# google-deepmind/bsuite

Hardware: AMD Instinct MI355X
Metric: env-steps/sec (higher is better)
Workload: dtype int32; 1 GPU; deep_sea/10 deep_sea {'size': 30, 'mapping_seed': 42} random actions, dense TimeStep; mode=e, lanes_per_gpu=1048576, global_lanes=1048576, episode_phases=staggered

## Files before the change

### bsuite_amd/csrc/deep_sea.hip

```cpp
#include "bsx_pair_host.h"
#include "bsx_tab_eval.h"
#include "deep_sea_fam.h"
#include "pair_mixed.h"

template <int K>
__global__ void __launch_bounds__(BSX_BLOCK) deep_sea_step1_kernel(const deep_sea_fam::args a, const uint32_t cells,
                                                                   const uint32_t cells_magic, const bsx_div64 dv) {
  __shared__ deep_sea_fam::shared s_map[BSX_BLOCK / BSX_WAVE];
  const int wl = (int)(threadIdx.x & 63u);
  deep_sea_fam::shared& map = s_map[threadIdx.x >> 6];
  const int64_t n_lanes = a.ctl.n_lanes;
  const uint64_t step = bsx_step_of(a.ctl);
  const int32_t tag_new = (int32_t)(((uint32_t)(step + 1) & 1u) << DS_TAG_SHIFT);
  const bool forced = a.ctl.force_reset != 0;
  const deep_sea_hot fn{a.size};
  const uint64_t total = (uint64_t)n_lanes * cells;
  const uint64_t F0 = (uint64_t)blockIdx.x * (uint64_t)(K * 4 * BSX_BLOCK);
  const uint64_t lane_b = __umul64hi(F0, dv.m) >> dv.s;
  const uint32_t r_b = (uint32_t)(F0 - lane_b * cells);
  bsx_f4* __restrict__ o4 = reinterpret_cast<bsx_f4*>(a.out.observation + F0);
  const int32_t* __restrict__ st_b = a.state + lane_b;
  const int32_t* __restrict__ act_b = a.action + (forced ? 0 : lane_b);

  uint32_t dl[K];
  int r0[K];
  bool live[K];
#pragma unroll
  for (int u = 0; u < K; ++u) {
    const uint32_t c = (threadIdx.x >> 6) * (K * 64) + u * 64 + (threadIdx.x & 63);
    const uint32_t f = r_b + (c << 2);
    dl[u] = __umulhi(f, cells_magic);
    r0[u] = (int)(f - dl[u] * cells);
    live[u] = F0 + ((uint64_t)c << 2) + 3 < total;
  }
  const uint32_t dA = dl[0];
  uint32_t dB = dA;
  bool wrA = false, wrB = false;
#pragma unroll
  for (int u = 0; u < K; ++u) {
    if (live[u]) dB = dl[u];
  }
#pragma unroll
  for (int u = 0; u < K; ++u) {
    wrA |= live[u] && r0[u] == 0 && dl[u] == dA;
    wrB |= live[u] && r0[u] == 0 && dl[u] == dB && dB != dA;
  }
  const bool any = live[0];
  const int32_t wA = any ? st_b[dA] : 0, wB = any ? st_b[dB] : 0;
  const int aA = (any && !forced) ? act_b[dA] : 0, aB = (any && !forced) ? act_b[dB] : 0;

  const int map_words = (a.size * a.size + 31) >> 5;
  static_assert(DS_MAP_WORDS <= 2 * BSX_WAVE, "the per-wave copy of the action mapping is two passes at most");
  if (wl < map_words) map.map[wl] = a.mapping_bits[wl];
  if (wl + BSX_WAVE < map_words) map.map[wl + BSX_WAVE] = a.mapping_bits[wl + BSX_WAVE];
  bsx_wave_sync();


  auto resolve = [&](uint32_t d, int32_t w, int act, bool writer, int& type) -> int32_t {
    type = -1;
    if (!writer && (w & DS_TAG_BIT) == tag_new) return w;
    const int64_t L = (int64_t)lane_b + d;
    int32_t nst; double reward;
    const int ty = deep_sea_fam::advance<true, 1>(a, map, L, a.ctl.lane_offset + (uint64_t)L, step, w, act, nst, reward, writer);
    if (writer) {
      type = ty;
      a.state[L] = nst;
      bsx_emit_at<0, 0, false>(a.ctl, a.out, L, L, a.ctl.lane_offset + (uint64_t)L, step, ty, reward);
    }
    return nst;
  };
  int tA = -1, tB = -1;
  int32_t nA = 0, nB = 0;
  if (any) {
    nA = resolve(dA, wA, aA, wrA, tA);
    nB = dB != dA ? resolve(dB, wB, aB, wrB, tB) : nA;
  }
  int hA, hB, unused;
  fn(nA, hA, unused);
  fn(nB, hB, unused);
#pragma unroll
  for (int u = 0; u < K; ++u) {
    if (!live[u]) continue;
    int hot = dl[u] == dA ? hA : hB;
    const int p0 = hot < 0 ? -1 : hot - r0[u];
    bsx_f4 v;
    v.x = p0 == 0 ? 1.0f : 0.0f;
    v.y = p0 == 1 ? 1.0f : 0.0f;
    v.z = p0 == 2 ? 1.0f : 0.0f;
    v.w = p0 == 3 ? 1.0f : 0.0f;
    o4[(threadIdx.x >> 6) * (K * 64) + u * 64 + (threadIdx.x & 63)] = v;
  }
  const unsigned int n_last = (unsigned int)__popcll(__ballot(tA == BSX_LAST)) + (unsigned int)__popcll(__ballot(tB == BSX_LAST));
  const unsigned int n_first = (unsigned int)__popcll(__ballot(tA == BSX_FIRST)) + (unsigned int)__popcll(__ballot(tB == BSX_FIRST));
  if (a.ctl.counters != nullptr && wl == 0 && (n_last | n_first) != 0u) {
    unsigned long long* shard = (unsigned long long*)a.ctl.counters +
                                (size_t)((blockIdx.x * (BSX_BLOCK / BSX_WAVE) + (threadIdx.x >> 6)) & (BSX_COUNTER_SHARDS - 1)) * BSX_COUNTER_STRIDE;
    if (n_last) atomicAdd(&shard[0], (unsigned long long)n_last);
    if (n_first) atomicAdd(&shard[1], (unsigned long long)n_first);
  }
}

static int deep_sea_check_cfg(const bsx_deep_sea_t* cfg) {
  return (cfg->size < 1 || cfg->size > BSX_DEEP_SEA_MAX_SIZE) ? BSX_ERANGE : 0;
}

static void deep_sea_fill(const bsx_deep_sea_t* cfg, const bsx_call_t* call, const int32_t* action, int32_t* state,
                          bsx_timestep_t out, double* info, deep_sea_fam::args* a) {
  a->ctl = bsx_make_ctl(call);
  a->action = action; a->state = state; a->out = out; a->info = info;
  a->move_cost = cfg->move_cost; a->inv_size = cfg->inv_size;
  a->size = cfg->size; a->deterministic = cfg->deterministic;
  for (int w = 0; w < DS_MAP_WORDS; ++w) a->mapping_bits[w] = cfg->mapping_bits[w];
}

static int deep_sea_make(const bsx_deep_sea_t* cfg, const bsx_call_t* call, const int32_t* action,
                         int32_t* state, bsx_timestep_t out, double* info, deep_sea_fam::args* a) {
  if (cfg == nullptr) return BSX_ENULL;
  int rc = bsx_check_call(call, action, out, true, true);
  if (rc != 0) return rc;
  if ((rc = deep_sea_check_cfg(cfg)) != 0) return rc;
  if (call->stream.mt_state != nullptr && !cfg->deterministic && call->stream.mt_gauss == nullptr)
    return BSX_ENULL;
  if (call->n_lanes > 0 && (state == nullptr || info == nullptr)) return BSX_ENULL;
  deep_sea_fill(cfg, call, action, state, out, info, a);
  return 0;
}

extern "C" int bsx_deep_sea_step(const bsx_deep_sea_t* cfg, const bsx_call_t* call,
                                 const int32_t* action, int32_t* state, bsx_timestep_t out,
                                 double* info) {
  deep_sea_fam::args a;
  int rc = deep_sea_make(cfg, call, action, state, out, info, &a);
  if (rc != 0) return rc;
  if (call->n_lanes == 0) return 0;
  const uint32_t cells = (uint32_t)(cfg->size * cfg->size);
  static const int step1_env = bsx_env_int("BSX_DEEP_SEA_STEP1", 1);
  if (step1_env != 0 && (int64_t)call->n_lanes * cells * 4 <= ((int64_t)1 << 30) && (call->flags & BSX_CALL_STATE_TAGGED) && call->n_steps <= 1 && call->action_ring <= 1 && cfg->deterministic && bsx_ctl_lean(a.ctl) &&
      call->obs_paint == nullptr && bsx_call_obs(call) == 0 && !bsx_call_index(call) && (cells & 3u) == 0 && cells >= 3u * 256u) {
    constexpr int K = 4;
    const uint64_t total = (uint64_t)call->n_lanes * cells;
    const uint64_t blocks = (total + (uint64_t)K * 4 * BSX_BLOCK - 1) / ((uint64_t)K * 4 * BSX_BLOCK);
    if (blocks > 0x7FFFFFFFull) return BSX_EINVAL;
    deep_sea_step1_kernel<K><<<dim3((unsigned)blocks), dim3(BSX_BLOCK), 0, (hipStream_t)call->hip_stream>>>(
        a, cells, bsx_div_magic(cells), bsx_make_div64(cells));
    return bsx_launch_status();
  }
  return bsx_pair_call<deep_sea_fam, deep_sea_hot, 4>(a, call, action, state, out, cells, deep_sea_hot{cfg->size});
}

extern "C" int bsx_deep_sea_policy_rollout(const bsx_deep_sea_t* cfg, const bsx_call_t* call, const bsx_policy_t* policy,
                                           int32_t* state, bsx_timestep_t out, double* info) {
  if (cfg == nullptr || call == nullptr || policy == nullptr) return BSX_ENULL;
  int rc = deep_sea_check_cfg(cfg);
  if (rc == 0) rc = bsx_check_policy_call(call, policy, bsx_policy_states_deep_sea(cfg->size), state, out, info);
  if (rc != 0 || call->n_lanes == 0) return rc;
  deep_sea_fam::args a;
  rc = deep_sea_make(cfg, call, policy->actions_out, state, out, info, &a);
  if (rc != 0) return rc;
  a.action = nullptr;
  return bsx_policy_rollout_call<deep_sea_fam, deep_sea_hot>(a, call, policy, 2u, out, deep_sea_hot{cfg->size});
}

extern "C" int bsx_deep_sea_policy_evaluate(const bsx_deep_sea_t* cfg, const bsx_call_t* call, const bsx_policy_t* policy,
                                             int32_t* state, bsx_policy_eval_t out, double* info) {
  if (cfg == nullptr || call == nullptr || policy == nullptr) return BSX_ENULL;
  int rc = deep_sea_check_cfg(cfg);
  if (rc == 0) rc = bsx_check_policy_eval_call(call, policy, bsx_policy_states_deep_sea(cfg->size), state, out, info);
  if (rc != 0 || call->n_lanes == 0) return rc;
  bsx_tab_eval_args e;
  deep_sea_fill(cfg, call, nullptr, state, bsx_timestep_t{}, info, &e.fam.deep_sea);
  return bsx_tab_eval_call(e, BSX_FAM_DEEP_SEA, call, policy, 2u, out);
}

extern "C" int bsx_group_set_deep_sea(bsx_group_t* g, int32_t index, const bsx_deep_sea_t* cfg,
                                      const bsx_call_t* call, const int32_t* action, int32_t* state,
                                      bsx_timestep_t out, double* info) {
  if (g == nullptr) return BSX_ENULL;
  if (call != nullptr && (bsx_call_obs(call) != 0 || bsx_call_index(call))) return BSX_EMODE;
  int rc;
  deep_sea_fam::args a;
  if (bsx_is_mixed_pair_group(g)) {
    rc = deep_sea_make(cfg, call, action, state, out, info, &a);
    if (rc != 0) return rc;
    a.ctl.state_in = call->state_alt;
    const uint32_t cells = (uint32_t)(cfg->size * cfg->size);
    if (cells < 4u) return BSX_ERANGE;
    const bsx_stream_seg<deep_sea_hot> sg = bsx_make_stream_seg(out.observation, state, a.ctl.n_lanes, cells, deep_sea_hot{cfg->size});
    return bsx_mixed_put(g, BSX_FAM_DEEP_SEA, index, call, &a, sizeof(a), &sg, sizeof(sg),
                              (uint64_t)bsx_blocks_of(a.ctl.n_lanes),
                              bsx_flat_blocks((uint64_t)a.ctl.n_lanes * cells, PAIR_DEEP_SEA_K), 0);
  }
  rc = bsx_group_check_set(g, BSX_FAM_DEEP_SEA, index, call, sizeof(deep_sea_fam::args),
                           sizeof(bsx_stream_seg<deep_sea_hot>), 0);
  if (rc != 0) return rc;
  rc = deep_sea_make(cfg, call, action, state, out, info, &a);
  if (rc != 0) return rc;
  g->launch = bsx_group_launch_pair<deep_sea_fam, deep_sea_hot, 4>;
  g->n_phases = 2;
  return bsx_group_put_pair<deep_sea_fam, deep_sea_hot>(g, index, a, out.observation, state,
                                                        (uint32_t)(cfg->size * cfg->size), deep_sea_hot{cfg->size}, 4);
}
```

### bsuite_amd/csrc/deep_sea_fam.h

```cpp
#ifndef BSX_DEEP_SEA_FAM_H_
#define BSX_DEEP_SEA_FAM_H_

#include "bsx_device.h"
#include "bsx_policy.h"

#define DS_RESET_BIT (1 << 17)
#define DS_TAG_SHIFT 18
#define DS_TAG_BIT (1 << DS_TAG_SHIFT)
#define DS_MAP_WORDS (BSX_DEEP_SEA_MAX_SIZE * BSX_DEEP_SEA_MAX_SIZE / 32)

struct deep_sea_fam {
  struct args {
    bsx_ctl ctl;
    const int32_t* action;
    int32_t* state;
    bsx_timestep_t out;
    double* info;
    double move_cost;
    double inv_size;
    int32_t size;
    int32_t deterministic;
    uint32_t mapping_bits[DS_MAP_WORDS];
  };
  struct shared { uint32_t map[DS_MAP_WORDS]; };

  __device__ static __forceinline__ void stage(const args& a, shared& s) {
    const int map_words = (a.size * a.size + 31) >> 5;
    for (int w = threadIdx.x; w < map_words; w += BSX_BLOCK) s.map[w] = a.mapping_bits[w];
  }

  template <bool LEAN = false, int DET = -1, bool NOMT = false>
  __device__ static __forceinline__ int advance(const args& a, const shared& s, int64_t i, uint64_t lane,
                                                uint64_t step, int32_t st, int act, int32_t& nst,
                                                double& reward, const bool commit = true) {
    BSX_NO_CONTRACT
    const int N = a.size;
    const bool deterministic = DET == 1 || a.deterministic;
    int row = st & 0xFF, col = (st >> 8) & 0xFF, bad = (st >> 16) & 1;
    int type;
    reward = 0.0;
    if (a.ctl.force_reset || (st & DS_RESET_BIT)) {
      row = 0; col = 0; bad = 0;
      type = BSX_FIRST;
    } else {
      const int cell = row * N + col;
      const int mapped = (int)((s.map[cell >> 5] >> (cell & 31)) & 1u);
      const bool right = (act == mapped);
      bsx_draws d;
      bsx_draws_begin<(LEAN || NOMT) ? 0 : -1>(&d, a.ctl, i, lane, step);
      if (col == N - 1 && right) {
        reward += 1.0;
        if (commit) a.info[a.ctl.n_lanes + i] += 1.0;
      }
      if (!deterministic && row == N - 1 && (col == 0 || col == N - 1))
        reward += bsx_normal(&d);
      if (right) {
        bool moves = true;
        if (!deterministic || (!LEAN && !NOMT && a.ctl.mt_state != nullptr)) {
          const double u = bsx_uniform(&d);
          moves = (u > a.inv_size) || deterministic;
        }
        if (moves) col = col + 1 > N - 1 ? N - 1 : col + 1;
        reward -= a.move_cost;
      } else {
        if (row == col) bad = 1;
        col = col - 1 < 0 ? 0 : col - 1;
      }
      bsx_draws_end<(LEAN || NOMT) ? 0 : -1>(&d, a.ctl, i);
      row += 1;
      if (row == N) {
        if (bad && commit) a.info[i] += 1.0;
        type = BSX_LAST;
      } else {
        type = BSX_MID;
      }
    }
    nst = row | (col << 8) | (bad << 16) | (type == BSX_LAST ? DS_RESET_BIT : 0) | (int32_t)(((uint32_t)(step + 1) & 1u) << DS_TAG_SHIFT);
    return type;
  }
  template <bool LEAN, bool NOMT>
  __device__ static __forceinline__ int advance_nomt(const args& a, const shared& s, int64_t i, uint64_t lane, uint64_t step,
                                                     int32_t st, int act, int32_t& nst, double& reward) {
    return advance<LEAN, -1, NOMT>(a, s, i, lane, step, st, act, nst, reward);
  }
  __device__ static __forceinline__ bool resets(int32_t st) { return (st & DS_RESET_BIT) != 0; }

  struct deferred { uint32_t bad, good; };
  __device__ static __forceinline__ int advance_deferred(const args& a, const shared& s, int64_t i, uint64_t lane, uint64_t step,
                                                         int32_t st, int act, int32_t& nst, double& reward, deferred& d) {
    const int type = advance<true>(a, s, i, lane, step, st, act, nst, reward, false);
    if (type != BSX_FIRST) {
      const int col = (st >> 8) & 0xFF, cell = (st & 0xFF) * a.size + col;
      const int mapped = (int)((s.map[cell >> 5] >> (cell & 31)) & 1u);
      d.good += (col == a.size - 1 && act == mapped) ? 1u : 0u;
      d.bad += (type == BSX_LAST && ((nst >> 16) & 1) != 0) ? 1u : 0u;
    }
    return type;
  }
  __device__ static __forceinline__ void commit_deferred(const args& a, int64_t i, const deferred& d) {
    if (d.bad != 0u) a.info[i] += (double)d.bad;
    if (d.good != 0u) a.info[a.ctl.n_lanes + i] += (double)d.good;
  }
};

struct deep_sea_hot {
  int N;
  static constexpr int INDEX_K = 1;
  static constexpr int FAMILY = BSX_FAM_DEEP_SEA;
  int geom0() const { return N; }
  int geom1() const { return 0; }
  __device__ __forceinline__ void operator()(int32_t st, int& a, int& b) const {
    const int row = st & 0xFF, col = (st >> 8) & 0xFF;
    a = row < N ? row * N + col : -1;
    b = -1;
  }
  __device__ __forceinline__ int policy_key(int32_t st) const {
    int a, b;
    (*this)(st, a, b);
    return bsx_policy_key_deep_sea(a);
  }
};

#endif
```

### bsuite_amd/environments/base.py

```python
import collections
import contextlib
import ctypes
import secrets
from typing import Any, Dict, Optional

import numpy as np
import torch

from bsuite_amd import _native
from bsuite_amd import dm_env_compat as dm_env
from bsuite_amd.dm_env_compat import specs

_MASK63 = (1 << 63) - 1


_current_raw_stream = getattr(torch._C, '_cuda_getCurrentRawStream', None)
if _current_raw_stream is None:
  def _current_raw_stream(index):
    return torch.cuda.current_stream(index).cuda_stream
_current_device = getattr(torch._C, '_cuda_getDevice', None) or torch.cuda.current_device


_OBS_CODES = {torch.float32: 0, torch.uint8: 1, torch.float16: 2, torch.bfloat16: 3}
_OBS_NAMES = {'float32': torch.float32, 'uint8': torch.uint8, 'float16': torch.float16, 'bfloat16': torch.bfloat16}
_OBS_SPEC_DTYPES = {torch.float32: np.float32, torch.uint8: np.uint8, torch.float16: np.float16,
                    torch.bfloat16: np.float32,
                    torch.int32: np.int32}


LOGGING_COLUMNS = ('steps', 'episode', 'total_return', 'episode_len', 'episode_return')

_MT_COLUMNS = ('state', 'pos', 'gauss', 'has_gauss')


PolicyEvaluation = collections.namedtuple('PolicyEvaluation', ['episodes', 'return_sum', 'episode_return_sum'])


def raw(env):
  return env.raw_env if hasattr(env, 'raw_env') else env


def _timestep_ptrs(o) -> '_native.TimeStepPtrs':
  return _native.TimeStepPtrs(o['reward'].data_ptr(), o['discount'].data_ptr(), o['step_type'].data_ptr(),
                              o['observation'].data_ptr())


def _resolve_seed(seed: Optional[int]) -> int:
  if seed is None:
    return secrets.randbits(63)
  return int(seed) & _MASK63


class Environment(dm_env.EnvironmentBase):

  bsuite_num_episodes: int

  _supports_delta = False
  _supports_narrow_obs = False
  _index_width = 0
  _pipelined_rollout = False
  scalar_host_buffers = True
  row_path_min_bytes = None
  _state_tag_bit = None
  _state_lib_bits = 0
  _tag_calls = False
  _info_keys = ()
  _info_int_keys = ()
  _abi_name = None
  _cfg = None

  def __init__(self, obs_shape, num_actions, *, seed=None, batch=None, device=None,
               lane_offset=0, num_buffers=2, device_step_counter=False, shared_step_counter=None,
               rng='philox', observation_mode='dense', obs_allocator=None, observation_dtype=torch.float32):
    self._scalar = batch is None
    self._scalar_last_type = None
    self._batch = 1 if batch is None else int(batch)
    if self._batch < 1:
      raise ValueError('batch must be >= 1')
    self._device = torch.device('cuda:0' if device is None else device)
    if self._device.type == 'cuda' and self._device.index is None:
      self._device = torch.device('cuda', torch.cuda.current_device() if torch.cuda.is_available() else 0)
    self._lane_offset = int(lane_offset)
    self._seed = _resolve_seed(seed if seed is None or isinstance(seed, (int, np.integer)) else 0)
    self._obs_shape = tuple(int(d) for d in obs_shape)
    self._num_actions = int(num_actions)
    self._num_buffers = max(1, int(num_buffers))
    self._device_step_counter = bool(device_step_counter) or shared_step_counter is not None
    self._shared_step_counter = shared_step_counter
    self._obs_allocator = obs_allocator
    self._resolve_observations(observation_mode, observation_dtype)
    if rng not in ('philox', 'mt19937'):
      raise ValueError("rng must be 'philox' or 'mt19937'")
    self._rng_mode = rng
    self._mt_seeds = None
    if rng == 'mt19937':
      if seed is None or isinstance(seed, (int, np.integer)):
        self._mt_seeds = [(self._seed + i) & 0xFFFFFFFF for i in range(self._batch)]
      else:
        self._mt_seeds = [int(x) for x in seed]
        if len(self._mt_seeds) != self._batch:
          raise ValueError('need one seed per lane')
    self._wrap = (_native.WRAP_NONE, 0.0, 0, 0.0)
    self._wrap_mt_seeds = None
    self._wrap_mt = None
    self._logging = None
    self._deferred_steps = None
    self._grouped_by = None
    self._rollout_out = {}
    self._policy_rollout_out = {}
    self._policy_eval_out = None
    self._state_alt = None
    self._row_buf = None
    self._dev_index = self._device.index
    self._step_index = 0
    self._buf = 0
    self._allocated = False
    self._reset_next_step = True

  def _resolve_observations(self, observation_mode, observation_dtype):
    if observation_mode not in ('dense', 'delta', 'index'):
      raise ValueError("observation_mode must be 'dense', 'delta' or 'index'")
    if observation_mode == 'delta' and not self._supports_delta:
      raise ValueError(f'{type(self).__name__} has no delta observation mode (its observations are small and dense)')
    self._delta = observation_mode == 'delta'
    self._index = observation_mode == 'index'
    self._board_shape = self._obs_shape
    if self._index:
      if not self._index_width:
        raise ValueError(f'{type(self).__name__} has no index observation mode (its observations are not one-hot boards)')
      if self._scalar:
        raise ValueError("observation_mode='index' needs the batched view (batch=B)")
      if self._obs_allocator is not None:
        raise ValueError("observation_mode='index' is not available in SweepBatch (float32 arenas)")
    dt = _OBS_NAMES.get(observation_dtype, observation_dtype) if isinstance(observation_dtype, str) else observation_dtype
    if dt not in _OBS_CODES:
      raise ValueError(f'observation_dtype must be one of {sorted(_OBS_NAMES)} (or the torch dtypes), got {observation_dtype!r}')
    if dt != torch.float32:
      if not self._supports_narrow_obs:
        raise ValueError(f'{type(self).__name__} writes float32 observations only (observation_dtype={observation_dtype!r})')
      if self._scalar:
        raise ValueError('observation_dtype other than float32 needs the batched view (batch=B)')
      if self._delta:
        raise ValueError("observation_dtype other than float32 needs observation_mode='dense'")
      if self._obs_allocator is not None:
        raise ValueError('observation_dtype other than float32 is not available in SweepBatch (float32 arenas)')
    if self._index and dt != torch.float32:
      raise ValueError("observation_mode='index' writes int32 cell numbers: observation_dtype must stay float32")
    self._obs_dtype = dt
    self._obs_flags = _OBS_CODES[dt] << _native.CALL_OBS_SHIFT
    if self._index:
      self._obs_shape, self._obs_dtype = (self._index_width,), torch.int32
      self._obs_flags = _native.CALL_OBS_INDEX

  @property
  def batch_size(self) -> int:
    return self._batch

  @property
  def device(self) -> torch.device:
    return self._device

  @property
  def seed(self) -> int:
    return self._seed

  @property
  def observation_dtype(self) -> torch.dtype:
    return self._obs_dtype

  @property
  def observation_mode(self) -> str:
    return 'index' if self._index else 'delta' if self._delta else 'dense'

  @property
  def board_shape(self):
    return self._board_shape

  @property
  def lane_offset(self) -> int:
    return self._lane_offset

  @property
  def step_index(self) -> int:
    return self._step_index

  def device_step_index(self) -> int:
    self._ensure_allocated()
    return int(self._step_base.item()) if self._device_step_counter else self._step_index

  @contextlib.contextmanager
  def step_counter_deferred(self):
    if not self._device_step_counter or self._shared_step_counter is not None:
      raise ValueError('step_counter_deferred() needs an environment built with device_step_counter=True')
    self._ensure_allocated()
    self._deferred_steps = 0
    try:
      yield self
    finally:
      n, self._deferred_steps = self._deferred_steps, None
      if n:
        with torch.cuda.device(self._device):
          _native.check(_native.lib.bsx_counter_add(self._step_base.data_ptr(), n,
                                                    torch.cuda.current_stream(self._device).cuda_stream),
                        'step counter bump')

  def _state_tensors(self) -> Dict[str, torch.Tensor]:
    raise NotImplementedError

  def _native_args(self, call, action_ptr, out):
    state = tuple(t.data_ptr() for t in self._state.values())
    info = (self._info.data_ptr(),) if self._info_keys else ()
    return (ctypes.byref(self._cfg), ctypes.byref(call), action_ptr) + state + (out,) + info

  def _launch(self, call, action_ptr, out) -> int:
    return getattr(_native.lib, f'bsx_{self._abi_name}_step')(*self._native_args(call, action_ptr, out))

  def _group_set(self, group, index: int, action: torch.Tensor, *, out=None, state_alt=None,
                 swap_state: bool = False, row_scratch=None) -> int:
    if self._index:
      raise ValueError("grouped launches write dense observations; use observation_mode='dense'")
    self._ensure_allocated()
    ring = int(action.shape[0]) if (torch.is_tensor(action) and action.dim() == 2) else 0
    if (not torch.is_tensor(action) or action.dtype != torch.int32 or action.device != self._device
        or tuple(action.shape) not in ((self._batch,), (ring, self._batch)) or not action.is_contiguous()
        or (action.dim() == 2 and (ring < 1 or ring & (ring - 1)))):
      raise ValueError(f'grouped launches read the action tensor in place every step: need a contiguous int32 '
                       f'tensor of shape ({self._batch},) — or an action ring (R, {self._batch}) with R a power '
                       f'of two — on {self._device}')
    if not self._device_step_counter:
      raise ValueError('grouped launches need device_step_counter / shared_step_counter')
    if self._delta:
      raise ValueError("grouped launches write dense observations; use observation_mode='dense'")
    if self._obs_flags:
      raise ValueError('grouped launches write float32 observations; use observation_dtype=torch.float32')
    call = self._call_desc
    call.force_reset, call.n_steps = 0, 0
    self._sync_wrap()
    call.stream.step_index = 0
    call.action_ring = ring
    self._buf = 1 % self._num_buffers
    ptrs = self._out_ptrs[0] if out is None else _timestep_ptrs(out)
    own = self._state.get('state')
    own_rows = call.row_scratch
    if row_scratch is not None:
      call.row_scratch = row_scratch.data_ptr() if row_scratch is not False else None
    try:
      if state_alt is not None:
        if swap_state:
          self._state['state'], call.state_alt = state_alt, own.data_ptr()
        else:
          call.state_alt = state_alt.data_ptr()
      return getattr(_native.lib, f'bsx_group_set_{self._abi_name}')(
          group, index, *self._native_args(call, action.data_ptr(), ptrs))
    finally:
      call.state_alt = None
      call.action_ring = 0
      call.row_scratch = own_rows
      if state_alt is not None:
        self._state['state'] = own

  def _row_scratch_words(self) -> int:
    fam = _native.FAMILY_IDS.get(self._abi_name, -1)
    return int(_native.lib.bsx_row_scratch_bytes(fam, int(np.prod(self._obs_shape)), self._batch)) // 4 if fam >= 0 else 0

  def _row_scratch(self, fresh: bool = False) -> Optional[torch.Tensor]:
    words = self._row_scratch_words()
    if not words:
      return None
    if fresh or self._row_buf is None:
      with torch.cuda.device(self._device):
        t = torch.empty(words, dtype=torch.int32, device=self._device)
      if fresh:
        return t
      self._row_buf = t
    return self._row_buf

  def _set_wrap_mt_seeds(self, seeds):
    self._wrap_mt_seeds = [int(s) & 0xFFFFFFFF for s in seeds]
    if self._allocated:
      self._upload_wrap_mt()

  @staticmethod
  def _mt_columns(seeds, device, prepare=None):
    B = len(seeds)
    keys = np.empty((B, 624), np.uint32)
    pos = np.empty(B, np.int32)
    gauss = np.zeros(B, np.float64)
    has = np.zeros(B, np.int32)
    for i, s_i in enumerate(seeds):
      rs = np.random.RandomState(s_i)
      if prepare is not None:
        prepare(rs)
      _, key, p, hg, cg = rs.get_state()
      keys[i], pos[i], has[i], gauss[i] = key, p, hg, cg
    cols = (np.ascontiguousarray(keys.T).view(np.int32), pos, gauss, has)
    return {k: torch.from_numpy(v).to(device) for k, v in zip(_MT_COLUMNS, cols)}

  def _upload_wrap_mt(self):
    with torch.cuda.device(self._device):
      self._wrap_mt = self._mt_columns(self._wrap_mt_seeds, self._device)
    for k, v in self._wrap_mt.items():
      setattr(self._call_desc.wrap, 'mt_' + k, v.data_ptr())

  def _mt_constructor_draws(self, rs: np.random.RandomState):
    """Subclass hook (rng='mt19937'): consume from `rs` exactly what the reference constructor
    draws from `self._rng` before the first reset (most families: nothing)."""

  def _ensure_allocated(self):
    if self._allocated:
      return
    if self._device.type != 'cuda' or not torch.cuda.is_available():
      raise RuntimeError(
          'bsuite_amd runs its environment dynamics in HIP kernels on an MI355X; no HIP device is '
          'visible to torch and there is deliberately no CPU fallback.')
    B, dev = self._batch, self._device
    with torch.cuda.device(dev):
      self._state = self._state_tensors()
      n_info = max(1, len(self._info_keys))
      self._info = torch.zeros((n_info, B), dtype=torch.float64, device=dev)
      self._counters = torch.zeros((_native.COUNTER_SHARDS, _native.COUNTER_STRIDE),
                                   dtype=torch.int64, device=dev)
      self._step_base = (self._shared_step_counter if self._shared_step_counter is not None
                         else torch.zeros(1, dtype=torch.int64, device=dev))
      self._host_out = self._scalar and self.scalar_host_buffers
      place = dict(pin_memory=True) if self._host_out else dict(device=dev)
      bufs = []
      for _ in range(self._num_buffers):
        obs = None
        if self._obs_allocator is not None and not self._scalar and not self._delta:
          obs = self._obs_allocator((B,) + self._obs_shape)
        elif self._delta:
          obs = torch.zeros((B,) + self._obs_shape, dtype=self._obs_dtype, **place)
        bufs.append(self._new_outputs((B,), place, obs))
      self._out, self._out_ptrs = [o for o, _, _ in bufs], [p for _, p, _ in bufs]
      self._timesteps = None if self._scalar else [ts for _, _, ts in bufs]
      self._paint = ([torch.full((B,), -1, dtype=torch.int32, device=dev) for _ in range(self._num_buffers)]
                     if self._delta else None)
      self._scalar_action = torch.zeros(1, dtype=torch.int32, **place)
      self._reward_f64 = torch.zeros(1, dtype=torch.float64, **place) if self._scalar else None
      self._out_np = [{k: v.numpy() for k, v in o.items()} for o in self._out] if self._host_out else None
    self._mt = None
    if self._rng_mode == 'mt19937':
      with torch.cuda.device(dev):
        self._mt = self._mt_columns(self._mt_seeds, dev, prepare=self._mt_constructor_draws)
    mt_ptrs = [self._mt[k].data_ptr() if self._mt else None for k in _MT_COLUMNS]
    self._call_desc = _native.Call(
        n_lanes=B, force_reset=0,
        stream=_native.Stream(self._seed, self._lane_offset, 0,
                              self._step_base.data_ptr() if self._device_step_counter else None,
                              *mt_ptrs),
        wrap=_native.RewardWrap(_native.WRAP_NONE, 0, 0.0, 0, None, None, None, None, 0.0),
        counters=self._counters.data_ptr(), hip_stream=None)
    if self._reward_f64 is not None:
      self._call_desc.reward_f64 = self._reward_f64.data_ptr()
    if (not self._scalar and self.row_path_min_bytes is not None and self._row_scratch_words()
        and B * int(np.prod(self._obs_shape)) * 4 >= self.row_path_min_bytes):
      self._call_desc.row_scratch = self._row_scratch().data_ptr()
    if self._wrap_mt_seeds is not None:
      self._upload_wrap_mt()
    self._fn = getattr(_native.lib, f'bsx_{self._abi_name}_step')
    self._family_id = _native.FAMILY_IDS[self._abi_name]
    self._reset_column = 'steps' if 'steps' in self._state else 'state'
    self._argv = [list(self._native_args(self._call_desc, 0, p)) for p in self._out_ptrs]
    self._call_stream, self._call_wrap = self._call_desc.stream, self._call_desc.wrap
    self._wrap_applied = None
    if self._state_tag_bit is not None:
      self._tag_calls = self._shared_step_counter is None
      self._call_desc.flags = _native.CALL_STATE_TAGGED if self._tag_calls else 0
    self._call_desc.flags |= self._obs_flags
    self._tag_host_count = self._tag_calls and not self._device_step_counter
    self._allocated = True

  def _new_outputs(self, lead, place, observation=None):
    o = dict(reward=torch.empty(lead, dtype=torch.float32, **place),
             discount=torch.empty(lead, dtype=torch.float32, **place),
             step_type=torch.empty(lead, dtype=torch.int8, **place),
             observation=(observation if observation is not None else
                          torch.empty(tuple(lead) + self._obs_shape, dtype=self._obs_dtype, **place)))
    return o, _timestep_ptrs(o), dm_env.TimeStep(step_type=o['step_type'], reward=o['reward'], discount=o['discount'],
                                                 observation=o['observation'])

  def _sync_wrap(self):
    w = self._call_desc.wrap
    w.kind, w.param, w.seed, w.param2 = self._wrap
    self._wrap_applied = self._wrap

  def _redirected(self, method, *args):
    with torch.cuda.device(self._device):
      return method(*args)

  def _call(self, action_ptr: int, force_reset: bool) -> int:
    if _current_device() != self._dev_index:
      return self._redirected(self._call, action_ptr, force_reset)
    b = self._buf
    self._buf = b + 1 if b + 1 < self._num_buffers else 0
    call = self._call_desc
    if self._delta:
      call.obs_paint = self._paint[b].data_ptr()
    call.force_reset = 1 if force_reset else 0
    if self._tag_host_count:
      call.flags = (0 if torch.cuda.is_current_stream_capturing() else _native.CALL_STATE_TAGGED) | self._obs_flags
    if self._wrap is not self._wrap_applied:
      w = self._call_wrap
      w.kind, w.param, w.seed, w.param2 = self._wrap
      self._wrap_applied = self._wrap
    hip_stream = _current_raw_stream(self._dev_index)
    call.hip_stream = hip_stream
    argv = self._argv[b]
    argv[2] = action_ptr
    if self._device_step_counter:
      if self._deferred_steps is not None:
        self._call_stream.step_index = self._deferred_steps
        rc = self._fn(*argv)
        self._call_stream.step_index = 0
        self._deferred_steps += 1
      else:
        rc = self._fn(*argv)
        if rc == 0 and self._shared_step_counter is None:
          rc = _native.lib.bsx_counter_add(self._step_base.data_ptr(), 1, hip_stream)
    else:
      self._call_stream.step_index = self._step_index
      rc = self._fn(*argv)
    if rc != 0:
      _native.check(rc, f'{type(self).__name__} step')
    self._step_index += 1
    return b

  def _launch_steps(self, fn, args, T: int, what: str):
    if _current_device() != self._dev_index:
      return self._redirected(self._launch_steps, fn, args, T, what)
    call = self._call_desc
    call.force_reset, call.n_steps = 0, T
    self._sync_wrap()
    hip_stream = _current_raw_stream(self._dev_index)
    call.hip_stream = hip_stream
    call.stream.step_index = 0 if self._device_step_counter else self._step_index
    try:
      rc = fn(*args)
      if rc == 0 and self._device_step_counter and self._shared_step_counter is None:
        rc = _native.lib.bsx_counter_add(self._step_base.data_ptr(), T, hip_stream)
    finally:
      call.n_steps = 0
      call.state_alt = None
    if rc != 0:
      _native.check(rc, f'{type(self).__name__} {what}')
    self._step_index += T
    return None

  def enable_logging(self, log_by_step: bool = False, log_every: bool = False,
                     max_rows: Optional[int] = None, max_count: Optional[int] = None):
    from bsuite_amd.utils import wrappers as _w
    if self._grouped_by is not None:
      raise RuntimeError('enable_logging() on a segment of prepared sweep groups: SweepBatch.release_groups() first')
    self._ensure_allocated()
    if self._logging is None:
      for j, pending in self._pending_info().items():
        self._info[j] += pending
      self._clear_pending_info()
    explicit_count = max_count is not None
    if max_count is None:
      max_count = 10 ** 18
    points = _w.logarithmic_logging_points(max_count)
    if max_rows is None:
      if self._scalar:
        max_rows = 8
      elif log_every:
        max_rows = 4096
      else:
        horizon = max_count if explicit_count else (
            max(10 ** 4, 100 * int(getattr(self, 'bsuite_num_episodes', 0) or 0)) * (1000 if log_by_step else 1))
        max_rows = (2 if log_by_step else 1) * sum(1 for p_ in points if p_ <= horizon) + 2
    B, dev = self._batch, self._device
    n_info = len(self._info_keys)
    place = dict(pin_memory=True) if self._host_out else dict(device=dev)
    lg = {k: torch.zeros(B, dtype=torch.float64 if k.endswith('_return') else torch.int64, **place)
          for k in LOGGING_COLUMNS}
    lg.update(rows=torch.zeros((B, max_rows, len(LOGGING_COLUMNS) + n_info), dtype=torch.float64, **place),
              n_rows=torch.zeros(B, dtype=torch.int32, **place),
              log_points=torch.tensor(points, dtype=torch.int64, device=dev))
    self._logging = lg
    self._logging_desc = _native.Logging(
        info=self._info.data_ptr() if n_info else None, **{k: v.data_ptr() for k, v in lg.items()},
        n_log_points=len(points), max_rows=max_rows,
        n_info=n_info, log_by_step=int(bool(log_by_step)), log_every=int(bool(log_every)))
    self._call_desc.logging = ctypes.pointer(self._logging_desc)
    return lg

  def logging_columns(self):
    return LOGGING_COLUMNS + tuple(self._info_keys)

  def _coerce_actions(self, action) -> torch.Tensor:
    if self._scalar:
      a = int(action)
      if self._scalar_last_type is not None and self._scalar_last_type != _native.LAST:
        self._check_scalar_action(a)
      if self._host_out:
        self._scalar_action.numpy()[0] = a
      else:
        self._scalar_action.fill_(a)
      return self._scalar_action
    if not torch.is_tensor(action):
      action = torch.as_tensor(np.asarray(action), device=self._device)
    if action.device != self._device:
      action = action.to(self._device)
    if action.dtype != torch.int32:
      action = action.to(torch.int32)
    if action.shape != (self._batch,):
      raise ValueError(f'expected actions of shape ({self._batch},), got {tuple(action.shape)}')
    return action.contiguous()

  def _check_scalar_action(self, action: int):
    """Scalar view only: subclasses raise what the reference raises for an invalid action."""

  def _wrap_output(self, b: int):
    if not self._scalar:
      return self._timesteps[b]
    out = self._out[b]
    if self._host_out:
      torch.cuda.current_stream(self._device).synchronize()
      o = self._out_np[b]
      st, reward, discount = int(o['step_type'][0]), float(self._reward_f64.numpy()[0]), float(o['discount'][0])
      obs = o['observation'][0].copy()
    else:
      st = int(out['step_type'].item())
      obs = out['observation'][0].cpu().numpy()
      reward, discount = float(self._reward_f64.item()), float(out['discount'].item())
    self._scalar_last_type = st
    if st == _native.FIRST:
      return dm_env.restart(obs)
    if st == _native.LAST:
      return dm_env.TimeStep(dm_env.StepType.LAST, reward, discount, obs)
    return dm_env.transition(reward=reward, observation=obs, discount=discount)

  def reset(self) -> dm_env.TimeStep:
    self._reset_next_step = False
    if not self._allocated:
      self._ensure_allocated()
    return self._wrap_output(self._call(0, force_reset=True))

  def step(self, action, reset_mask=None) -> dm_env.TimeStep:
    if not self._allocated:
      if reset_mask is not None:
        self._check_reset_mask(reset_mask)
      self._ensure_allocated()
    if reset_mask is None and (
        type(action) is torch.Tensor and action.dtype is torch.int32 and action.is_cuda and action.dim() == 1
        and action.size(0) == self._batch and action.is_contiguous() and action.get_device() == self._dev_index
        and not self._scalar):
      ptr = action.data_ptr()
    else:
      if reset_mask is not None:
        self._check_reset_mask(reset_mask)
      ptr = self._coerce_actions(action).data_ptr()
      if reset_mask is not None:
        self._mark_reset(reset_mask)
    return self._wrap_output(self._call(ptr, force_reset=False))

  def _check_reset_mask(self, mask):
    if self._scalar:
      raise ValueError('reset_mask / mark_reset() need the batched view (batch=B); reset() is the one lane of the '
                       'scalar view')
    if self._grouped_by is not None:
      raise RuntimeError('mark_reset() on a segment of prepared sweep groups: SweepBatch.release_groups() first')
    if (not torch.is_tensor(mask) or mask.dtype not in (torch.bool, torch.uint8) or mask.device != self._device
        or tuple(mask.shape) != (self._batch,) or not mask.is_contiguous()):
      raise ValueError(f'reset_mask must be a contiguous bool or uint8 tensor of shape ({self._batch},) on '
                       f'{self._device}')

  def _mark_reset(self, mask):
    if _current_device() != self._dev_index:
      return self._redirected(self._mark_reset, mask)
    col = self._info_pending_column
    folded = 1 if (self._logging is None and col is not None) else 0
    rc = _native.lib.bsx_lane_reset_mark(
        self._family_id, self._info_variant, self._batch, mask.data_ptr(),
        self._state[self._reset_column].data_ptr(), self._info.data_ptr(), folded, _current_raw_stream(self._dev_index))
    if rc != 0:
      _native.check(rc, f'{type(self).__name__} mark_reset')
    return None

  def mark_reset(self, mask):
    self._check_reset_mask(mask)
    self._ensure_allocated()
    self._mark_reset(mask)

  def rollout(self, actions) -> dm_env.TimeStep:
    if self._scalar:
      raise TypeError('rollout() needs the batched view (batch=B)')
    if self._delta:
      raise ValueError("rollout() writes T separate observation arrays; use observation_mode='dense'")
    self._ensure_allocated()
    if not torch.is_tensor(actions) or actions.dim() != 2 or actions.shape[1] != self._batch:
      raise ValueError(f'expected actions of shape (T, {self._batch})')
    if actions.device != self._device or actions.dtype != torch.int32:
      actions = actions.to(device=self._device, dtype=torch.int32)
    actions = actions.contiguous()
    T = int(actions.shape[0])
    if T < 1:
      raise ValueError('rollout needs at least one step')
    if T not in self._rollout_out:
      self._rollout_out[T] = self._new_outputs((T, self._batch), dict(device=self._device))
    _, ptrs, timestep = self._rollout_out[T]
    call = self._call_desc
    if self._pipelined_rollout and T > 1 and not self._index:
      if self._state_alt is None:
        self._state_alt = torch.empty_like(self._state['state'])
      call.state_alt = self._state_alt.data_ptr()
    self._launch_steps(self._fn, self._native_args(call, actions.data_ptr(), ptrs), T, 'rollout')
    return timestep

  _policy_abi = None

  @property
  def policy_num_states(self) -> int:
    raise ValueError(f'{type(self).__name__} has no tabular policy rollout (deep_sea and catch only)')

  def _check_rollout_policy(self, policy, num_steps, policy_index, epsilon, explore_seed, what='rollout_policy'):
    name = type(self).__name__
    if self._policy_abi is None:
      raise ValueError(f'{name} has no tabular policy rollout (deep_sea and catch only)')
    if self._scalar:
      raise ValueError(f'{what}() needs the batched view (batch=B)')
    if not self._index:
      raise ValueError(f"{what}() looks its actions up by the index observation: build the environment with "
                       f"observation_mode='index' (this one is {self.observation_mode!r}, {self._obs_dtype})")
    if self._rng_mode != 'philox':
      raise ValueError(f"{what}() needs the counter-based draw stream (rng='philox')")
    if self._logging is not None:
      raise ValueError(f'{what}() is not available with Logging enabled')
    if self._wrap[0] != _native.WRAP_NONE:
      raise ValueError(f'{what}() is not available under a reward wrapper')
    if self._grouped_by is not None:
      raise RuntimeError(f'{what}() on a segment of prepared sweep groups: SweepBatch.release_groups() first')
    if isinstance(num_steps, bool) or not isinstance(num_steps, (int, np.integer)) or num_steps < 1:
      raise ValueError(f'{what}: num_steps must be an integer >= 1, got {num_steps!r}')
    if isinstance(epsilon, bool) or not isinstance(epsilon, (int, float, np.integer, np.floating)) or not 0.0 <= float(epsilon) <= 1.0:
      raise ValueError(f'{what}: epsilon must be a number in [0, 1], got {epsilon!r}')
    if isinstance(explore_seed, bool) or not isinstance(explore_seed, (int, np.integer)) or not 0 <= int(explore_seed) < (1 << 64):
      raise ValueError(f'{what}: explore_seed must be an integer in [0, 2^64), got {explore_seed!r}')
    S = self.policy_num_states
    if (not torch.is_tensor(policy) or policy.dtype != torch.uint8 or policy.device != self._device or policy.dim() not in (1, 2)
        or int(policy.shape[-1]) != S or policy.numel() == 0 or not policy.is_contiguous()):
      raise ValueError(f'{what}: policy must be a contiguous uint8 tensor of shape ({S},) or (P, {S}) on {self._device}')
    P = 1 if policy.dim() == 1 else int(policy.shape[0])
    if P == 1:
      if policy_index is not None:
        raise ValueError(f'{what}: policy_index names the row of a population of tables; with one table it must be None')
    elif (not torch.is_tensor(policy_index) or policy_index.dtype != torch.int32 or policy_index.device != self._device
          or tuple(policy_index.shape) != (self._batch,) or not policy_index.is_contiguous()):
      raise ValueError(f'{what}: a population of {P} tables needs policy_index, a contiguous int32 tensor of shape '
                       f'({self._batch},) on {self._device}')
    return P

  def rollout_policy(self, policy, num_steps, *, policy_index=None, epsilon=0.0, explore_seed=0):
    P = self._check_rollout_policy(policy, num_steps, policy_index, epsilon, explore_seed)
    self._ensure_allocated()
    T = int(num_steps)
    if T not in self._policy_rollout_out:
      actions = torch.empty((T, self._batch), dtype=torch.int32, device=self._device)
      self._policy_rollout_out[T] = self._new_outputs((T, self._batch), dict(device=self._device)) + (actions,)
    _, ptrs, timestep, actions = self._policy_rollout_out[T]
    pol = _native.Policy(policy.data_ptr(), self.policy_num_states, P,
                         policy_index.data_ptr() if policy_index is not None else None,
                         float(epsilon), int(explore_seed), actions.data_ptr())
    args = (ctypes.byref(self._cfg), ctypes.byref(self._call_desc), ctypes.byref(pol), self._state['state'].data_ptr(), ptrs,
            self._info.data_ptr())
    self._launch_steps(getattr(_native.lib, self._policy_abi), args, T, 'rollout_policy')
    return timestep, actions

  _policy_eval_abi = None

  def evaluate_policy(self, policy, num_steps, *, policy_index=None, epsilon=0.0, explore_seed=0):
    P = self._check_rollout_policy(policy, num_steps, policy_index, epsilon, explore_seed, what='evaluate_policy')
    self._ensure_allocated()
    if self._policy_eval_out is None:
      self._policy_eval_out = PolicyEvaluation(
          episodes=torch.empty(self._batch, dtype=torch.int32, device=self._device),
          return_sum=torch.empty(self._batch, dtype=torch.float64, device=self._device),
          episode_return_sum=torch.empty(self._batch, dtype=torch.float64, device=self._device))
    ev = self._policy_eval_out
    pol = _native.Policy(policy.data_ptr(), self.policy_num_states, P,
                         policy_index.data_ptr() if policy_index is not None else None, float(epsilon), int(explore_seed), None)
    out = _native.PolicyEvalPtrs(ev.episodes.data_ptr(), ev.return_sum.data_ptr(), ev.episode_return_sum.data_ptr())
    args = (ctypes.byref(self._cfg), ctypes.byref(self._call_desc), ctypes.byref(pol), self._state['state'].data_ptr(), out,
            self._info.data_ptr())
    self._launch_steps(getattr(_native.lib, self._policy_eval_abi), args, int(num_steps), 'evaluate_policy')
    return ev

  def _step(self, action):
    raise NotImplementedError('The batched engine fuses _step/_reset into one kernel; call step().')

  def _reset(self):
    raise NotImplementedError('The batched engine fuses _step/_reset into one kernel; call reset().')

  def observation_spec(self):
    if self._index:
      return specs.BoundedArray(shape=self._obs_shape, dtype=np.int32, name='observation', minimum=-1,
                                maximum=int(np.prod(self._board_shape)) - 1)
    return specs.Array(shape=self._obs_shape, dtype=self._obs_spec_dtype(), name='observation')

  def _obs_spec_dtype(self):
    return _OBS_SPEC_DTYPES[self._obs_dtype]

  def action_spec(self):
    return specs.DiscreteArray(self._num_actions, name='action')

  def _pending_info(self) -> Dict[int, torch.Tensor]:
    return {}

  def _clear_pending_info(self):
    """Subclass hook: called once `_pending_info()` has been added to the columns (enable_logging), for families
    that keep the pending amount in state bits of their own (catch) rather than deriving it from a step counter."""

  _info_pending_column = None
  _info_variant = 0

  def _info_columns(self) -> torch.Tensor:
    if self._logging is not None or self._info_pending_column is None:
      return self._info
    cols = torch.empty_like(self._info)
    with torch.cuda.device(self._device):
      _native.check(_native.lib.bsx_bsuite_info(
          _native.FAMILY_IDS[self._abi_name], self._info_variant, self._batch,
          self._state[self._info_pending_column].data_ptr(), self._info.data_ptr(), self._info.shape[0], 1,
          cols.data_ptr(), torch.cuda.current_stream(self._device).cuda_stream), 'bsx_bsuite_info')
    return cols

  def bsuite_info(self) -> Dict[str, Any]:
    self._ensure_allocated()
    info = self._info_columns()
    if self._scalar:
      vals = info[:, 0].cpu().numpy()
      out = {}
      for j, k in enumerate(self._info_keys):
        if not k.startswith('_'):
          out[k] = int(vals[j]) if k in self._info_int_keys else float(vals[j])
      return out
    return {k: info[j] for j, k in enumerate(self._info_keys) if not k.startswith('_')}

  def episode_counters(self) -> torch.Tensor:
    self._ensure_allocated()
    return self._counters[:, :2].sum(dim=0)

  def invalid_action_count(self) -> torch.Tensor:
    self._ensure_allocated()
    return self._counters[:, 2].sum()

  def state_dict(self) -> Dict[str, Any]:
    self._ensure_allocated()
    d = {k: v.clone() for k, v in self._state.items()}
    if self._state_lib_bits:
      d['state'] &= ~self._state_lib_bits
    d['__info'] = self._info.clone()
    d['__counters'] = self._counters.clone()
    d['__step_index'] = self.device_step_index()
    d['__seed'] = self._seed
    if self._rng_mode == 'mt19937':
      for k, v in self._mt.items():
        d['__mt_' + k] = v.clone()
      if self._wrap_mt is not None:
        for k, v in self._wrap_mt.items():
          d['__wrap_mt_' + k] = v.clone()
    d['__wrap'] = tuple(self._wrap)
    if self._logging is not None:
      for k in LOGGING_COLUMNS + ('rows', 'n_rows'):
        d['__logging_' + k] = self._logging[k].clone()
    return d

  def load_state_dict(self, d: Dict[str, Any]):
    self._ensure_allocated()
    self._scalar_last_type = None
    for k, v in self._state.items():
      v.copy_(d[k])
    self._info.copy_(d['__info'])
    self._counters.copy_(d['__counters'])
    self._step_index = int(d['__step_index'])
    if self._state_tag_bit is not None:
      st = self._state['state']
      st &= ~self._state_lib_bits
      if self._step_index & 1:
        st |= self._state_tag_bit
    if self._device_step_counter:
      self._step_base.fill_(self._step_index)
    self._seed = int(d['__seed'])
    self._call_desc.stream.seed = self._seed
    if self._rng_mode == 'mt19937':
      for k, v in self._mt.items():
        v.copy_(d['__mt_' + k])
      if self._wrap_mt is not None:
        for k, v in self._wrap_mt.items():
          v.copy_(d['__wrap_mt_' + k])
    if '__wrap' in d:
      self._wrap = (tuple(d['__wrap']) + (0.0,))[:4]
    has_log = '__logging_steps' in d
    if has_log != (self._logging is not None):
      raise ValueError('state_dict was taken %s the Logging wrapper but this environment runs %s it: '
                       'wrap (or unwrap) the environment before load_state_dict'
                       % (('with', 'without') if has_log else ('without', 'with')))
    if has_log:
      if d['__logging_rows'].shape != self._logging['rows'].shape:
        raise ValueError('Logging row buffers differ in shape (max_rows): construct Logging with the same max_rows')
      for k in LOGGING_COLUMNS + ('rows', 'n_rows'):
        self._logging[k].copy_(d['__logging_' + k])
```

### bsuite_amd/environments/deep_sea.py

```python
import warnings
from typing import Optional

import numpy as np
import torch

from bsuite_amd import _native
from bsuite_amd.environments import base

NUM_EPISODES = 10000


class DeepSea(base.Environment):

  _info_keys = ('total_bad_episodes', 'denoised_return')
  _info_int_keys = ('total_bad_episodes',)

  def __init__(self,
               size: int,
               deterministic: bool = True,
               unscaled_move_cost: float = 0.01,
               randomize_actions: bool = True,
               seed: Optional[int] = None,
               mapping_seed: Optional[int] = None,
               **engine_kwargs):
    if not 1 <= size <= _native.DEEP_SEA_MAX_SIZE:
      raise ValueError(f'size must be in [1, {_native.DEEP_SEA_MAX_SIZE}]')
    super().__init__(obs_shape=(size, size), num_actions=2, seed=seed, **engine_kwargs)
    self._size = size
    self._deterministic = deterministic
    self._unscaled_move_cost = unscaled_move_cost

    if randomize_actions:
      self._mapping_rng = np.random.RandomState(mapping_seed)
      self._action_mapping = self._mapping_rng.binomial(1, 0.5, [size, size])
    else:
      warnings.warn('Environment is in debug mode (randomize_actions=False).'
                    'Only randomized_actions=True is the DeepSea environment.')
      self._action_mapping = np.ones([size, size])

    if not self._deterministic:
      optimal_no_cost = (1 - 1 / self._size) ** (self._size - 1)
    else:
      optimal_no_cost = 1.
    self._optimal_return = optimal_no_cost - self._unscaled_move_cost

    cfg = _native.DeepSeaCfg()
    cfg.size = size
    cfg.deterministic = int(bool(deterministic))
    cfg.move_cost = float(unscaled_move_cost) / size
    cfg.inv_size = 1 / size
    flat = np.asarray(self._action_mapping).reshape(-1) == 1
    for idx in np.nonzero(flat)[0]:
      cfg.mapping_bits[int(idx) >> 5] |= (1 << (int(idx) & 31))
    self._cfg = cfg
    self.bsuite_num_episodes = NUM_EPISODES

  def _state_tensors(self):
    return dict(state=torch.full((self._batch,), 1 << 17, dtype=torch.int32, device=self._device))

  _abi_name = 'deep_sea'
  _supports_delta = True
  _supports_narrow_obs = True
  _index_width = 1
  _pipelined_rollout = True

  _state_tag_bit = 1 << 18
  _state_lib_bits = 1 << 18

  _policy_abi = 'bsx_deep_sea_policy_rollout'
  _policy_eval_abi = 'bsx_deep_sea_policy_evaluate'

  @property
  def policy_num_states(self) -> int:
    return self._size * self._size

  @property
  def optimal_return(self):
    return self._optimal_return
```

Baseline: 1.769 billion env-steps/s.

## Cache action-mapping bit in state word and inline deep_sea step1 update

Stores the mapping bit for the agent's current cell in bit 19 of the state word, so the step can resolve the action direction without reading the mapping table. The one-hot cell for the observation is computed directly from the old state, and the next cell's mapping bit is fetched from registers with ds_bpermute, which removes the per-wave shared-memory copy and wave sync. The writer-lane state and timestep update is inlined and moved after the observation stores. In exchange the state layout changes, the generic advance path must write the bit too, and load_state_dict has to rebuild it on the host.

```diff
diff --git a/bsuite_amd/csrc/deep_sea.hip b/bsuite_amd/csrc/deep_sea.hip
--- a/bsuite_amd/csrc/deep_sea.hip
+++ b/bsuite_amd/csrc/deep_sea.hip
@@ -6,14 +6,12 @@
 template <int K>
 __global__ void __launch_bounds__(BSX_BLOCK) deep_sea_step1_kernel(const deep_sea_fam::args a, const uint32_t cells,
                                                                    const uint32_t cells_magic, const bsx_div64 dv) {
-  __shared__ deep_sea_fam::shared s_map[BSX_BLOCK / BSX_WAVE];
   const int wl = (int)(threadIdx.x & 63u);
-  deep_sea_fam::shared& map = s_map[threadIdx.x >> 6];
+  const int N = a.size;
   const int64_t n_lanes = a.ctl.n_lanes;
   const uint64_t step = bsx_step_of(a.ctl);
   const int32_t tag_new = (int32_t)(((uint32_t)(step + 1) & 1u) << DS_TAG_SHIFT);
   const bool forced = a.ctl.force_reset != 0;
-  const deep_sea_hot fn{a.size};
   const uint64_t total = (uint64_t)n_lanes * cells;
   const uint64_t F0 = (uint64_t)blockIdx.x * (uint64_t)(K * 4 * BSX_BLOCK);
   const uint64_t lane_b = __umul64hi(F0, dv.m) >> dv.s;
@@ -49,47 +47,85 @@
   const int32_t wA = any ? st_b[dA] : 0, wB = any ? st_b[dB] : 0;
   const int aA = (any && !forced) ? act_b[dA] : 0, aB = (any && !forced) ? act_b[dB] : 0;
 
-  const int map_words = (a.size * a.size + 31) >> 5;
-  static_assert(DS_MAP_WORDS <= 2 * BSX_WAVE, "the per-wave copy of the action mapping is two passes at most");
-  if (wl < map_words) map.map[wl] = a.mapping_bits[wl];
-  if (wl + BSX_WAVE < map_words) map.map[wl + BSX_WAVE] = a.mapping_bits[wl + BSX_WAVE];
-  bsx_wave_sync();
-
-
-  auto resolve = [&](uint32_t d, int32_t w, int act, bool writer, int& type) -> int32_t {
-    type = -1;
-    if (!writer && (w & DS_TAG_BIT) == tag_new) return w;
+  const int map_words = (N * N + 31) >> 5;
+  static_assert(DS_MAP_WORDS <= 2 * BSX_WAVE, "two mapping words per lane at most");
+  const uint32_t mlo = wl < map_words ? a.mapping_bits[wl] : 0u;
+  const uint32_t mhi = wl + BSX_WAVE < map_words ? a.mapping_bits[wl + BSX_WAVE] : 0u;
+  auto hot_of = [&](int32_t w, int act, bool writer) -> int {
+    const int row = w & 0xFF, col = (w >> 8) & 0xFF;
+    const bool advanced = !writer && (w & DS_TAG_BIT) == tag_new;
+    const bool reset = forced || (w & DS_RESET_BIT) != 0;
+    const bool right = act == ((w >> DS_RIGHT_SHIFT) & 1);
+    int ncol = col + (right ? 1 : -1);
+    ncol = ncol < 0 ? 0 : (ncol > N - 1 ? N - 1 : ncol);
+    int nrow = row + 1;
+    if (reset) { nrow = 0; ncol = 0; }
+    if (advanced) { nrow = row; ncol = col; }
+    return nrow < N ? nrow * N + ncol : -1;
+  };
+  const int hA = hot_of(wA, aA, wrA);
+  const int hB = dB != dA ? hot_of(wB, aB, wrB) : hA;
+  int32_t rbA, rbB;
+  {
+    const uint32_t iA = hA >= 0 ? (uint32_t)hA >> 5 : 0u, iB = hB >= 0 ? (uint32_t)hB >> 5 : 0u;
+    uint32_t mA = (uint32_t)__builtin_amdgcn_ds_bpermute((int)((iA & 63u) << 2), (int)mlo);
+    uint32_t mB = (uint32_t)__builtin_amdgcn_ds_bpermute((int)((iB & 63u) << 2), (int)mlo);
+    if (map_words > BSX_WAVE) {
+      const uint32_t xA = (uint32_t)__builtin_amdgcn_ds_bpermute((int)((iA & 63u) << 2), (int)mhi);
+      const uint32_t xB = (uint32_t)__builtin_amdgcn_ds_bpermute((int)((iB & 63u) << 2), (int)mhi);
+      mA = iA >= 64u ? xA : mA;
+      mB = iB >= 64u ? xB : mB;
+    }
+    rbA = (int32_t)((mA >> (hA & 31)) & 1u) << DS_RIGHT_SHIFT;
+    rbB = (int32_t)((mB >> (hB & 31)) & 1u) << DS_RIGHT_SHIFT;
+  }
+
+  auto publish = [&](uint32_t d, int32_t w, int act, int32_t right_of_new) -> int {
+    BSX_NO_CONTRACT
     const int64_t L = (int64_t)lane_b + d;
-    int32_t nst; double reward;
-    const int ty = deep_sea_fam::advance<true, 1>(a, map, L, a.ctl.lane_offset + (uint64_t)L, step, w, act, nst, reward, writer);
-    if (writer) {
-      type = ty;
-      a.state[L] = nst;
-      bsx_emit_at<0, 0, false>(a.ctl, a.out, L, L, a.ctl.lane_offset + (uint64_t)L, step, ty, reward);
+    int row = w & 0xFF, col = (w >> 8) & 0xFF, bad = (w >> 16) & 1;
+    int type;
+    bool good = false;
+    double reward = 0.0;
+    if (forced || (w & DS_RESET_BIT)) {
+      row = 0; col = 0; bad = 0;
+      type = BSX_FIRST;
+    } else {
+      const bool right = act == ((w >> DS_RIGHT_SHIFT) & 1);
+      good = col == N - 1 && right;
+      if (good) reward += 1.0;
+      if (right) {
+        col = col + 1 > N - 1 ? N - 1 : col + 1;
+        reward -= a.move_cost;
+      } else {
+        if (row == col) bad = 1;
+        col = col - 1 < 0 ? 0 : col - 1;
+      }
+      row += 1;
+      type = row == N ? BSX_LAST : BSX_MID;
     }
-    return nst;
+    a.state[L] = row | (col << 8) | (bad << 16) | (type == BSX_LAST ? DS_RESET_BIT : 0) | tag_new | (type == BSX_LAST ? 0 : right_of_new);
+    bsx_emit_at<0, 0, false>(a.ctl, a.out, L, L, a.ctl.lane_offset + (uint64_t)L, step, type, reward);
+    if (good) a.info[n_lanes + L] += 1.0;
+    if (type == BSX_LAST && bad) a.info[L] += 1.0;
+    return type;
   };
   int tA = -1, tB = -1;
-  int32_t nA = 0, nB = 0;
-  if (any) {
-    nA = resolve(dA, wA, aA, wrA, tA);
-    nB = dB != dA ? resolve(dB, wB, aB, wrB, tB) : nA;
-  }
-  int hA, hB, unused;
-  fn(nA, hA, unused);
-  fn(nB, hB, unused);
-#pragma unroll
-  for (int u = 0; u < K; ++u) {
-    if (!live[u]) continue;
-    int hot = dl[u] == dA ? hA : hB;
-    const int p0 = hot < 0 ? -1 : hot - r0[u];
-    bsx_f4 v;
-    v.x = p0 == 0 ? 1.0f : 0.0f;
-    v.y = p0 == 1 ? 1.0f : 0.0f;
-    v.z = p0 == 2 ? 1.0f : 0.0f;
-    v.w = p0 == 3 ? 1.0f : 0.0f;
-    o4[(threadIdx.x >> 6) * (K * 64) + u * 64 + (threadIdx.x & 63)] = v;
-  }
+#pragma unroll
+  for (int u = 0; u < K; ++u) {
+    if (live[u]) {
+      int hot = dl[u] == dA ? hA : hB;
+      const int p0 = hot < 0 ? -1 : hot - r0[u];
+      bsx_f4 v;
+      v.x = p0 == 0 ? 1.0f : 0.0f;
+      v.y = p0 == 1 ? 1.0f : 0.0f;
+      v.z = p0 == 2 ? 1.0f : 0.0f;
+      v.w = p0 == 3 ? 1.0f : 0.0f;
+      o4[(threadIdx.x >> 6) * (K * 64) + u * 64 + (threadIdx.x & 63)] = v;
+    }
+  }
+  if (wrA) tA = publish(dA, wA, aA, rbA);
+  if (wrB) tB = publish(dB, wB, aB, rbB);
   const unsigned int n_last = (unsigned int)__popcll(__ballot(tA == BSX_LAST)) + (unsigned int)__popcll(__ballot(tB == BSX_LAST));
   const unsigned int n_first = (unsigned int)__popcll(__ballot(tA == BSX_FIRST)) + (unsigned int)__popcll(__ballot(tB == BSX_FIRST));
   if (a.ctl.counters != nullptr && wl == 0 && (n_last | n_first) != 0u) {
@@ -100,6 +136,8 @@
   }
 }
 
+#define DS_STEP1_MAX_BYTES ((int64_t)1 << 30)
+
 static int deep_sea_check_cfg(const bsx_deep_sea_t* cfg) {
   return (cfg->size < 1 || cfg->size > BSX_DEEP_SEA_MAX_SIZE) ? BSX_ERANGE : 0;
 }
@@ -135,7 +173,7 @@
   if (call->n_lanes == 0) return 0;
   const uint32_t cells = (uint32_t)(cfg->size * cfg->size);
   static const int step1_env = bsx_env_int("BSX_DEEP_SEA_STEP1", 1);
-  if (step1_env != 0 && (int64_t)call->n_lanes * cells * 4 <= ((int64_t)1 << 30) && (call->flags & BSX_CALL_STATE_TAGGED) && call->n_steps <= 1 && call->action_ring <= 1 && cfg->deterministic && bsx_ctl_lean(a.ctl) &&
+  if (step1_env != 0 && (int64_t)call->n_lanes * cells * 4 <= DS_STEP1_MAX_BYTES && (call->flags & BSX_CALL_STATE_TAGGED) && call->n_steps <= 1 && call->action_ring <= 1 && cfg->deterministic && bsx_ctl_lean(a.ctl) &&
       call->obs_paint == nullptr && bsx_call_obs(call) == 0 && !bsx_call_index(call) && (cells & 3u) == 0 && cells >= 3u * 256u) {
     constexpr int K = 4;
     const uint64_t total = (uint64_t)call->n_lanes * cells;
diff --git a/bsuite_amd/csrc/deep_sea_fam.h b/bsuite_amd/csrc/deep_sea_fam.h
--- a/bsuite_amd/csrc/deep_sea_fam.h
+++ b/bsuite_amd/csrc/deep_sea_fam.h
@@ -7,6 +7,8 @@
 #define DS_RESET_BIT (1 << 17)
 #define DS_TAG_SHIFT 18
 #define DS_TAG_BIT (1 << DS_TAG_SHIFT)
+#define DS_RIGHT_SHIFT 19
+#define DS_RIGHT_BIT (1 << DS_RIGHT_SHIFT)
 #define DS_MAP_WORDS (BSX_DEEP_SEA_MAX_SIZE * BSX_DEEP_SEA_MAX_SIZE / 32)
 
 struct deep_sea_fam {
@@ -75,7 +77,12 @@
         type = BSX_MID;
       }
     }
-    nst = row | (col << 8) | (bad << 16) | (type == BSX_LAST ? DS_RESET_BIT : 0) | (int32_t)(((uint32_t)(step + 1) & 1u) << DS_TAG_SHIFT);
+    int32_t right_of_new = 0;
+    if (type != BSX_LAST) {
+      const int ncell = row * N + col;
+      right_of_new = (int32_t)((s.map[ncell >> 5] >> (ncell & 31)) & 1u) << DS_RIGHT_SHIFT;
+    }
+    nst = row | (col << 8) | (bad << 16) | (type == BSX_LAST ? DS_RESET_BIT : 0) | (int32_t)(((uint32_t)(step + 1) & 1u) << DS_TAG_SHIFT) | right_of_new;
     return type;
   }
   template <bool LEAN, bool NOMT>
diff --git a/bsuite_amd/environments/base.py b/bsuite_amd/environments/base.py
--- a/bsuite_amd/environments/base.py
+++ b/bsuite_amd/environments/base.py
@@ -64,6 +64,9 @@
   _state_tag_bit = None
   _state_lib_bits = 0
   _tag_calls = False
+
+  def _state_word_bits(self, st: torch.Tensor):
+    """load_state_dict: rebuilds in place whatever `_state_lib_bits` holds besides the tag (deep_sea: bit 19)."""
   _info_keys = ()
   _info_int_keys = ()
   _abi_name = None
@@ -780,6 +783,7 @@
       st &= ~self._state_lib_bits
       if self._step_index & 1:
         st |= self._state_tag_bit
+      self._state_word_bits(st)
     if self._device_step_counter:
       self._step_base.fill_(self._step_index)
     self._seed = int(d['__seed'])
diff --git a/bsuite_amd/environments/deep_sea.py b/bsuite_amd/environments/deep_sea.py
--- a/bsuite_amd/environments/deep_sea.py
+++ b/bsuite_amd/environments/deep_sea.py
@@ -65,7 +65,18 @@
   _pipelined_rollout = True
 
   _state_tag_bit = 1 << 18
-  _state_lib_bits = 1 << 18
+  _state_lib_bits = 3 << 18
+
+  @staticmethod
+  def right_bits(state: torch.Tensor, mapping: torch.Tensor, size: int) -> torch.Tensor:
+    row, col = state & 0xFF, (state >> 8) & 0xFF
+    inside = (row < size) & ((state & (1 << 17)) == 0)
+    cell = torch.where(inside, row * size + col, torch.zeros_like(row)).long().clamp_(max=size * size - 1)
+    return torch.where(inside, mapping[cell].to(state.dtype) << 19, torch.zeros_like(state))
+
+  def _state_word_bits(self, st: torch.Tensor):
+    mapping = torch.from_numpy(np.asarray(self._action_mapping).reshape(-1) == 1).to(st.device)
+    st |= self.right_bits(st, mapping, self._size)
 
   _policy_abi = 'bsx_deep_sea_policy_rollout'
   _policy_eval_abi = 'bsx_deep_sea_policy_evaluate'
```

Result: no change. 1.781 billion env-steps/s (median of 2 runs) (+0.7%).
